# francescofugazzi/3dgsconverter

Hardware: NVIDIA H100
Metric: Msplats/s SOR k=16 (higher is better)
Workload: dtype f32

## Files before the change

### 3dgsconverter_b200/csrc/gsx_sor.cu

```cuda
#include "gsx_common.cuh"
#include "gsx_sor.cuh"

#include "gsx_radix.cuh"
#include <math.h>

namespace gsx {

#define GSX_D2LIM_BITS 0x60ad78ebu
#define GSX_FULL 0xffffffffu

constexpr int kMortonBits = 15;
constexpr float kMortonScale = (float)(1 << (kMortonBits / 3));
constexpr float kMortonMax = kMortonScale - 1.f;
constexpr int kSmallBucket = 64;
constexpr int kQueryBatch = 16;
constexpr int kMergeThreshold = 9;
constexpr int kKnnMinBlocks = 8;
constexpr int kFlatSupers = 8;
const char* sor_build_info() {
    return "knn=r02c;epi_smem=1;first_sort=1;query_batch=16;minblocks=8;merge_threshold=9;small_bucket=64;"
           "flat_supers=8;knn16=0;tma=0;i32=1";
}


SorWs sor_carve(void* ws, int64_t ws_bytes, int64_t n, size_t sort_ws_bytes) {
    SorWs w;
    Carver c(ws, (size_t)ws_bytes);
    int64_t nchunk = (n + 31) / 32, nsuper = (nchunk + 31) / 32;
    w.n = n;
    w.spos = c.take<float4>(n);
    w.tab_se = c.take<int2>(n);
    w.tab_box = c.take<float4>(2 * n);
    w.startbits = c.take<uint32_t>(nchunk);
    w.cellbits = c.take<uint32_t>(nchunk);
    w.bigbits = c.take<uint32_t>(nchunk);
    w.startlist = c.take<uint32_t>(n / 8 + 1024);
    w.caabb = c.take<float4>(2 * nchunk);
    w.saabb = c.take<float4>(2 * nsuper);
    w.partial = c.take<float>(6 * 1024);
    w.minmax = c.take<float>(8);
    w.counters = c.take<unsigned int>(64);
    w.stats = c.take<unsigned long long>(8);
    w.meanstd = c.take<float>(8);
    w.ms_bytes = mean_std_ws_bytes(n);
    w.ms_ws = c.take<char>(w.ms_bytes);
    w.grid_total = align_up(c.off, 256);
    w.keys0 = c.take<uint64_t>(n);
    w.keys1 = c.take<uint64_t>(n);
    w.sort_ws_bytes = sort_ws_bytes;
    w.sort_ws = c.take<char>(sort_ws_bytes);
    w.total = align_up(c.off, 256);
    w.ok = c.ok();
    w.grid_ok = w.grid_total <= (size_t)(ws_bytes > 0 ? ws_bytes : 0);
    return w;
}

size_t sor_sort_ws_bytes(int64_t n) { return radix_ws_bytes(n) + 256; }

int64_t sor_workspace_bytes(int64_t n) {
    if (n < 1) n = 1;
    SorWs w = sor_carve(nullptr, 0, n, sor_sort_ws_bytes(n));
    return (int64_t)w.total + 1024;
}

int64_t sor_grid_workspace_bytes(int64_t n) {
    if (n < 1) n = 1;
    SorWs w = sor_carve(nullptr, 0, n, sor_sort_ws_bytes(n));
    return (int64_t)w.grid_total;
}


__global__ void __launch_bounds__(256) k_minmax_partial(const float* __restrict__ xyz, int64_t n,
                                                        float* __restrict__ partial) {
    float lo[3] = {INFINITY, INFINITY, INFINITY}, hi[3] = {-INFINITY, -INFINITY, -INFINITY};
    int64_t stride = (int64_t)gridDim.x * blockDim.x;
    for (int64_t i = (int64_t)blockIdx.x * blockDim.x + threadIdx.x; i < n; i += stride) {
#pragma unroll
        for (int a = 0; a < 3; ++a) {
            float v = xyz[3 * i + a];
            lo[a] = fminf(lo[a], v);
            hi[a] = fmaxf(hi[a], v);
        }
    }
    __shared__ float sm[6][8];
#pragma unroll
    for (int a = 0; a < 3; ++a) {
#pragma unroll
        for (int o = 16; o > 0; o >>= 1) {
            lo[a] = fminf(lo[a], __shfl_xor_sync(GSX_FULL, lo[a], o));
            hi[a] = fmaxf(hi[a], __shfl_xor_sync(GSX_FULL, hi[a], o));
        }
        if (lane_id() == 0) {
            sm[a][threadIdx.x >> 5] = lo[a];
            sm[3 + a][threadIdx.x >> 5] = hi[a];
        }
    }
    __syncthreads();
    if (threadIdx.x < 6) {
        float r = sm[threadIdx.x][0];
        for (int w = 1; w < 8; ++w) r = threadIdx.x < 3 ? fminf(r, sm[threadIdx.x][w]) : fmaxf(r, sm[threadIdx.x][w]);
        partial[blockIdx.x * 6 + threadIdx.x] = r;
    }
}

__global__ void k_minmax_final(const float* __restrict__ partial, int nblocks, float* __restrict__ out) {
    const int a = threadIdx.x >> 5, lane = threadIdx.x & 31;
    if (a >= 6) return;
    float r = a < 3 ? INFINITY : -INFINITY;
    for (int b = lane; b < nblocks; b += 32) r = a < 3 ? fminf(r, partial[b * 6 + a]) : fmaxf(r, partial[b * 6 + a]);
#pragma unroll
    for (int o = 16; o > 0; o >>= 1) {
        float t = __shfl_xor_sync(GSX_FULL, r, o);
        r = a < 3 ? fminf(r, t) : fmaxf(r, t);
    }
    if (lane == 0) out[a] = r;
}

int sor_minmax(const float* xyz, int64_t n, float* minmax_dev, float* partial, cudaStream_t st) {
    int blocks = (int)((n + 255) / 256);
    int cap = sm_count() * 4;
    if (blocks > cap) blocks = cap;
    if (blocks > 1024) blocks = 1024;
    if (blocks < 1) blocks = 1;
    k_minmax_partial<<<blocks, 256, 0, st>>>(xyz, n, partial);
    GSX_KERNEL_CHECK();
    k_minmax_final<<<1, 192, 0, st>>>(partial, blocks, minmax_dev);
    GSX_KERNEL_CHECK();
    return GSX_OK;
}


__device__ __forceinline__ uint32_t spread6(uint32_t v) {
    v &= 63u;
    v = (v | (v << 8)) & 0x0000300Fu;
    v = (v | (v << 4)) & 0x000030C3u;
    v = (v | (v << 2)) & 0x00009249u;
    return v;
}

__device__ __forceinline__ uint32_t bucket_hash(float x, float y, float z, float bx, float by, float bz, float cell,
                                                int64_t n, uint64_t M64, float& fx, float& fy, float& fz, float& flx,
                                                float& fly, float& flz) {
    fx = __fdiv_rn(__fsub_rn(x, bx), cell);
    fy = __fdiv_rn(__fsub_rn(y, by), cell);
    fz = __fdiv_rn(__fsub_rn(z, bz), cell);
    flx = floorf(fx), fly = floorf(fy), flz = floorf(fz);
    int64_t gx = (int64_t)(int32_t)flx, gy = (int64_t)(int32_t)fly, gz = (int64_t)(int32_t)flz;
    int64_t hx = (gx * 73856093LL) ^ (gy * 19349663LL) ^ (gz * 83492791LL);
    int64_t h;
    if (hx >= 0) {
        uint64_t q = __umul64hi((uint64_t)hx, M64);
        uint64_t r = (uint64_t)hx - q * (uint64_t)n;
        while (r >= (uint64_t)n) r -= (uint64_t)n;
        h = (int64_t)r;
    } else {
        h = hx % n;
        if (h < 0) h += n;
    }
    return (uint32_t)h;
}

__device__ __forceinline__ uint32_t bucket_of(float x, float y, float z, float bx, float by, float bz, float cell,
                                              int64_t n, uint64_t M64) {
    float a, b, c, d, e, f;
    return bucket_hash(x, y, z, bx, by, bz, cell, n, M64, a, b, c, d, e, f);
}

__device__ __forceinline__ uint64_t bucket_key(float x, float y, float z, float bx, float by, float bz, float cell,
                                               int64_t n, uint64_t M64) {
    float fx, fy, fz, flx, fly, flz;
    const uint32_t h = bucket_hash(x, y, z, bx, by, bz, cell, n, M64, fx, fy, fz, flx, fly, flz);
    uint32_t sx = (uint32_t)fminf(kMortonMax, fmaxf(0.f, (fx - flx) * kMortonScale));
    uint32_t sy = (uint32_t)fminf(kMortonMax, fmaxf(0.f, (fy - fly) * kMortonScale));
    uint32_t sz = (uint32_t)fminf(kMortonMax, fmaxf(0.f, (fz - flz) * kMortonScale));
    uint32_t mort = (spread6(sx) << 2) | (spread6(sy) << 1) | spread6(sz);
    return ((uint64_t)h << kMortonBits) | (uint64_t)mort;
}

struct PackFmt {
    int idx_bits, mort_bits, bucket_bits;
    __host__ __device__ int key_shift() const { return idx_bits + mort_bits; }
    __host__ __device__ uint64_t idx_mask() const { return (1ull << idx_bits) - 1ull; }
    __host__ __device__ int sort_begin() const { return idx_bits; }
    __host__ __device__ int sort_end() const { return idx_bits + mort_bits + bucket_bits; }
};

static int bits_for(int64_t n) {
    int b = 1;
    while (((int64_t)1 << b) < n) ++b;
    return b;
}

static PackFmt pack_fmt(int64_t n_items, int64_t n_buckets) {
    PackFmt f;
    f.idx_bits = bits_for(n_items);
    f.bucket_bits = bits_for(n_buckets);
    int avail = 64 - f.idx_bits - f.bucket_bits;
    if (avail > kMortonBits) avail = kMortonBits;
    f.mort_bits = avail < 0 ? 0 : avail - avail % 3;
    return f;
}

__device__ __forceinline__ uint64_t pack_word(uint64_t key , uint64_t bucket_sub,
                                              int64_t idx, PackFmt f) {
    const uint64_t bucket = (key >> kMortonBits) - bucket_sub;
    const uint64_t mort = (key & ((1ull << kMortonBits) - 1ull)) >> (kMortonBits - f.mort_bits);
    return (((bucket << f.mort_bits) | mort) << f.idx_bits) | (uint64_t)idx;
}

__global__ void __launch_bounds__(256) k_sor_keys(const float* __restrict__ xyz, int64_t n, float bx, float by,
                                                  float bz, float cell, uint64_t M64, PackFmt f,
                                                  uint64_t* __restrict__ keys) {
    int64_t i = (int64_t)blockIdx.x * blockDim.x + threadIdx.x;
    if (i >= n) return;
    keys[i] = pack_word(bucket_key(xyz[3 * i], xyz[3 * i + 1], xyz[3 * i + 2], bx, by, bz, cell, n, M64), 0, i, f);
}

__device__ __forceinline__ uint32_t float_to_ord(float f) {
    const uint32_t u = __float_as_uint(f);
    return (u & 0x80000000u) ? ~u : (u | 0x80000000u);
}
__device__ __forceinline__ float ord_to_float(uint32_t o) {
    return __uint_as_float((o & 0x80000000u) ? (o & 0x7fffffffu) : ~o);
}

template <bool GATHER>
__device__ __forceinline__ void
    sor_finish_tile(const int64_t tile, const float* __restrict__ xyz, const uint64_t* __restrict__ keys, PackFmt fmt,
                    float4* __restrict__ spos, int64_t n, float bx, float by, float bz, float cell, uint64_t M64,
                    int2* __restrict__ tab_se, uint32_t* __restrict__ startbits, uint32_t* __restrict__ cellbits,
                    float4* __restrict__ caabb, float4* __restrict__ saabb) {
    const int64_t j = tile * 1024 + threadIdx.x;
    const int lane = lane_id();
    float lo[3] = {INFINITY, INFINITY, INFINITY}, hi[3] = {-INFINITY, -INFINITY, -INFINITY};
    uint32_t h = 0xffffffffu;
    auto hash_at = [&](int64_t t) -> uint32_t {
        if (GATHER) return (uint32_t)(keys[t] >> fmt.key_shift());
        const float4 q = spos[t];
        return bucket_of(q.x, q.y, q.z, bx, by, bz, cell, n, M64);
    };
    int gcx = 0x7fffffff, gcy = 0, gcz = 0;
    if (j < n) {
        float x, y, z;
        if (GATHER) {
            const uint64_t word = keys[j];
            const int32_t idx = (int32_t)(word & fmt.idx_mask());
            x = xyz[3 * (int64_t)idx], y = xyz[3 * (int64_t)idx + 1], z = xyz[3 * (int64_t)idx + 2];
            spos[j] = make_float4(x, y, z, __int_as_float(idx));
            h = (uint32_t)(word >> fmt.key_shift());
        } else {
            const float4 p = spos[j];
            x = p.x, y = p.y, z = p.z;
            h = bucket_of(x, y, z, bx, by, bz, cell, n, M64);
        }
        gcx = (int)floorf(__fdiv_rn(__fsub_rn(x, bx), cell));
        gcy = (int)floorf(__fdiv_rn(__fsub_rn(y, by), cell));
        gcz = (int)floorf(__fdiv_rn(__fsub_rn(z, bz), cell));
        lo[0] = hi[0] = x;
        lo[1] = hi[1] = y;
        lo[2] = hi[2] = z;
    }
    __shared__ uint32_t sh_h[1024];
    sh_h[threadIdx.x] = h;
    __syncthreads();
    uint32_t hprev = threadIdx.x > 0 ? sh_h[threadIdx.x - 1] : 0xffffffffu;
    uint32_t hnext = threadIdx.x < 1023 ? sh_h[threadIdx.x + 1] : 0xffffffffu;
    if (j < n) {
        if (threadIdx.x == 0 && j > 0) hprev = hash_at(j - 1);
        if (threadIdx.x == 1023 && j + 1 < n) hnext = hash_at(j + 1);
    }
    __shared__ int sh_c[3][1024];
    sh_c[0][threadIdx.x] = gcx, sh_c[1][threadIdx.x] = gcy, sh_c[2][threadIdx.x] = gcz;
    __syncthreads();
    const bool newcell = j < n && (threadIdx.x == 0 || sh_c[0][threadIdx.x - 1] != gcx ||
                                   sh_c[1][threadIdx.x - 1] != gcy || sh_c[2][threadIdx.x - 1] != gcz);
    const unsigned cb = __ballot_sync(GSX_FULL, newcell);
    const bool start = j < n && (j == 0 || h != hprev);
    const bool end = j < n && (j == n - 1 || h != hnext);
    if (start) tab_se[h].x = (int)j;
    if (end) tab_se[h].y = (int)(j + 1);
    const unsigned sb = __ballot_sync(GSX_FULL, start);
#pragma unroll
    for (int a = 0; a < 3; ++a) {
        lo[a] = ord_to_float(__reduce_min_sync(GSX_FULL, float_to_ord(lo[a])));
        hi[a] = ord_to_float(__reduce_max_sync(GSX_FULL, float_to_ord(hi[a])));
    }
    __shared__ float sm[6][32];
    const int w = threadIdx.x >> 5;
    const int64_t chunk = tile * 32 + w;
    if (lane == 0) {
        if (chunk * 32 < n) {
            startbits[chunk] = sb;
            cellbits[chunk] = cb;
            caabb[2 * chunk] = make_float4(lo[0], lo[1], lo[2], hi[0]);
            caabb[2 * chunk + 1] = make_float4(hi[1], hi[2], 0.f, 0.f);
        }
        for (int a = 0; a < 3; ++a) {
            sm[a][w] = lo[a];
            sm[3 + a][w] = hi[a];
        }
    }
    __syncthreads();
    if (w == 0) {
        float v[6];
#pragma unroll
        for (int a = 0; a < 6; ++a) {
            v[a] = sm[a][lane];
#pragma unroll
            for (int o = 16; o > 0; o >>= 1) {
                float t = __shfl_xor_sync(GSX_FULL, v[a], o);
                v[a] = a < 3 ? fminf(v[a], t) : fmaxf(v[a], t);
            }
        }
        if (lane == 0) {
            saabb[2 * tile] = make_float4(v[0], v[1], v[2], v[3]);
            saabb[2 * tile + 1] = make_float4(v[4], v[5], 0.f, 0.f);
        }
    }
}

template <bool GATHER>
__global__ void __launch_bounds__(1024)
    k_sor_finish(const float* __restrict__ xyz, const uint64_t* __restrict__ keys, PackFmt fmt,
                 float4* __restrict__ spos, int64_t n, float bx, float by, float bz, float cell, uint64_t M64,
                 int2* __restrict__ tab_se, uint32_t* __restrict__ startbits, uint32_t* __restrict__ cellbits,
                 float4* __restrict__ caabb, float4* __restrict__ saabb) {
    sor_finish_tile<GATHER>(blockIdx.x, xyz, keys, fmt, spos, n, bx, by, bz, cell, M64, tab_se, startbits, cellbits, caabb,
                            saabb);
}

__global__ void __launch_bounds__(1024)
    k_sor_finish_gated(float4* __restrict__ spos, int64_t n, float bx, float by, float bz, float cell, uint64_t M64,
                       int2* __restrict__ tab_se, uint32_t* __restrict__ startbits, uint32_t* __restrict__ cellbits,
                       float4* __restrict__ caabb, float4* __restrict__ saabb, const unsigned int* __restrict__ gate) {
    if (!*gate) return;
    const int64_t tiles = (n + 1023) / 1024;
    for (int64_t t = blockIdx.x; t < tiles; t += gridDim.x) {
        sor_finish_tile<false>(t, nullptr, nullptr, PackFmt{}, spos, n, bx, by, bz, cell, M64, tab_se, startbits, cellbits,
                               caabb, saabb);
        __syncthreads();
    }
}

__device__ __forceinline__ void bucket_box_partial(const float4* __restrict__ spos, const float4* __restrict__ caabb,
                                                   int64_t s, int64_t end, int lane, float (&lo)[3], float (&hi)[3]) {
    lo[0] = lo[1] = lo[2] = INFINITY;
    hi[0] = hi[1] = hi[2] = -INFINITY;
    int64_t cf = (s + 31) >> 5, cl = end >> 5;
    int64_t head_end = cf * 32, tail_begin = cl * 32;
    if (cf > cl) {
        head_end = end;
        tail_begin = end;
        cf = cl = 0;
    }
    for (int64_t t = s + lane; t < head_end; t += 32) {
        float4 p = spos[t];
        lo[0] = fminf(lo[0], p.x), lo[1] = fminf(lo[1], p.y), lo[2] = fminf(lo[2], p.z);
        hi[0] = fmaxf(hi[0], p.x), hi[1] = fmaxf(hi[1], p.y), hi[2] = fmaxf(hi[2], p.z);
    }
    for (int64_t c = cf + lane; c < cl; c += 32) {
        float4 a = caabb[2 * c], b = caabb[2 * c + 1];
        lo[0] = fminf(lo[0], a.x), lo[1] = fminf(lo[1], a.y), lo[2] = fminf(lo[2], a.z);
        hi[0] = fmaxf(hi[0], a.w), hi[1] = fmaxf(hi[1], b.x), hi[2] = fmaxf(hi[2], b.y);
    }
    for (int64_t t = tail_begin + lane; t < end; t += 32) {
        float4 p = spos[t];
        lo[0] = fminf(lo[0], p.x), lo[1] = fminf(lo[1], p.y), lo[2] = fminf(lo[2], p.z);
        hi[0] = fmaxf(hi[0], p.x), hi[1] = fmaxf(hi[1], p.y), hi[2] = fmaxf(hi[2], p.z);
    }
}

__device__ __forceinline__ void
    bucket_boxes_chunk(const int64_t chunk, const uint32_t* __restrict__ startbits, const float4* __restrict__ spos,
                       const float4* __restrict__ caabb, const int2* __restrict__ tab_se, int64_t n, float bx,
                       float by, float bz, float cell, uint64_t M64, float4* __restrict__ tab_box) {
    const int lane = lane_id();
    if (chunk * 32 >= n) return;
    unsigned m = startbits[chunk];
    uint32_t my_h = 0;
    int my_end = 0;
    if ((m >> lane) & 1u) {
        const float4 p0 = spos[chunk * 32 + lane];
        my_h = bucket_of(p0.x, p0.y, p0.z, bx, by, bz, cell, n, M64);
        my_end = tab_se[my_h].y;
    }
    while (m) {
        const int src = __ffs(m) - 1;
        m &= m - 1;
        const int64_t s = chunk * 32 + src;
        const uint32_t hb = __shfl_sync(GSX_FULL, my_h, src);
        const int64_t end = __shfl_sync(GSX_FULL, my_end, src);
        float lo[3], hi[3];
        bucket_box_partial(spos, caabb, s, end, lane, lo, hi);
#pragma unroll
        for (int a = 0; a < 3; ++a)
#pragma unroll
            for (int o = 16; o > 0; o >>= 1) {
                lo[a] = fminf(lo[a], __shfl_xor_sync(GSX_FULL, lo[a], o));
                hi[a] = fmaxf(hi[a], __shfl_xor_sync(GSX_FULL, hi[a], o));
            }
        if (lane == 0) {
            tab_box[2 * (size_t)hb] = make_float4(lo[0], lo[1], lo[2], 0.f);
            tab_box[2 * (size_t)hb + 1] = make_float4(hi[0], hi[1], hi[2], 0.f);
        }
    }
}

__global__ void __launch_bounds__(256)
    k_sor_bucket_boxes(const uint32_t* __restrict__ startbits, const float4* __restrict__ spos,
                       const float4* __restrict__ caabb, const int2* __restrict__ tab_se, int64_t n, float bx,
                       float by, float bz, float cell, uint64_t M64, float4* __restrict__ tab_box) {
    bucket_boxes_chunk(((int64_t)blockIdx.x * blockDim.x + threadIdx.x) >> 5, startbits, spos, caabb, tab_se, n, bx, by, bz,
                       cell, M64, tab_box);
}

__global__ void __launch_bounds__(256)
    k_sor_bucket_boxes_gated(const uint32_t* __restrict__ startbits, const float4* __restrict__ spos,
                             const float4* __restrict__ caabb, const int2* __restrict__ tab_se, int64_t n, float bx,
                             float by, float bz, float cell, uint64_t M64, float4* __restrict__ tab_box,
                             const unsigned int* __restrict__ gate) {
    if (!*gate) return;
    const int64_t nchunk = (n + 31) >> 5, step = ((int64_t)gridDim.x * blockDim.x) >> 5;
    for (int64_t c = ((int64_t)blockIdx.x * blockDim.x + threadIdx.x) >> 5; c < nchunk; c += step)
        bucket_boxes_chunk(c, startbits, spos, caabb, tab_se, n, bx, by, bz, cell, M64, tab_box);
}

struct StartList {
    unsigned int* count;
    unsigned int* pos;
    unsigned int capacity;
};

__global__ void __launch_bounds__(1024)
    k_sor_finish_flags(const float4* __restrict__ spos, const uint8_t* __restrict__ flags, int64_t n,
                       uint32_t* __restrict__ startbits, uint32_t* __restrict__ cellbits, float4* __restrict__ caabb,
                       float4* __restrict__ saabb, StartList sl) {
    const int64_t j = (int64_t)blockIdx.x * 1024 + threadIdx.x;
    const int lane = lane_id();
    float lo[3] = {INFINITY, INFINITY, INFINITY}, hi[3] = {-INFINITY, -INFINITY, -INFINITY};
    bool start = false, newcell = false;
    if (j < n) {
        const float4 p = spos[j];
        lo[0] = hi[0] = p.x;
        lo[1] = hi[1] = p.y;
        lo[2] = hi[2] = p.z;
        const uint8_t f = flags[j];
        start = (f & 1) != 0;
        newcell = (f & 2) != 0;
    }
    const unsigned sb = __ballot_sync(GSX_FULL, start), cb = __ballot_sync(GSX_FULL, newcell);
    __shared__ unsigned s_wcnt[32], s_base;
    const int w = threadIdx.x >> 5;
    if (lane == 0) s_wcnt[w] = __popc(sb);
#pragma unroll
    for (int a = 0; a < 3; ++a) {
        lo[a] = ord_to_float(__reduce_min_sync(GSX_FULL, float_to_ord(lo[a])));
        hi[a] = ord_to_float(__reduce_max_sync(GSX_FULL, float_to_ord(hi[a])));
    }
    __shared__ float sm[6][32];
    const int64_t chunk = (int64_t)blockIdx.x * 32 + w;
    if (lane == 0) {
        if (chunk * 32 < n) {
            startbits[chunk] = sb;
            cellbits[chunk] = cb;
            caabb[2 * chunk] = make_float4(lo[0], lo[1], lo[2], hi[0]);
            caabb[2 * chunk + 1] = make_float4(hi[1], hi[2], 0.f, 0.f);
        }
        for (int a = 0; a < 3; ++a) {
            sm[a][w] = lo[a];
            sm[3 + a][w] = hi[a];
        }
    }
    __syncthreads();
    if (w == 0) {
        unsigned v = s_wcnt[lane], x = v;
#pragma unroll
        for (int o = 1; o < 32; o <<= 1) {
            unsigned y = __shfl_up_sync(GSX_FULL, x, o);
            if (lane >= o) x += y;
        }
        s_wcnt[lane] = x - v;
        if (lane == 31) {
            unsigned base = 0;
            if (x) {
                base = atomicAdd(sl.count, x);
                if (base + x > sl.capacity) {
                    atomicExch(sl.count + 1, 1u);
                    base = 0xffffffffu;
                }
            }
            s_base = base;
        }
        float vb[6];
#pragma unroll
        for (int a = 0; a < 6; ++a) {
            vb[a] = sm[a][lane];
#pragma unroll
            for (int o = 16; o > 0; o >>= 1) {
                float t = __shfl_xor_sync(GSX_FULL, vb[a], o);
                vb[a] = a < 3 ? fminf(vb[a], t) : fmaxf(vb[a], t);
            }
        }
        if (lane == 0) {
            saabb[2 * (int64_t)blockIdx.x] = make_float4(vb[0], vb[1], vb[2], vb[3]);
            saabb[2 * (int64_t)blockIdx.x + 1] = make_float4(vb[4], vb[5], 0.f, 0.f);
        }
    }
    __syncthreads();
    if (start && s_base != 0xffffffffu)
        sl.pos[s_base + s_wcnt[w] + __popc(sb & ((1u << lane) - 1u))] = (unsigned)j;
}

__global__ void __launch_bounds__(256)
    k_sor_bucket_tail(const float4* __restrict__ spos, const uint8_t* __restrict__ flags, int64_t n, float bx, float by,
                      float bz, float cell, uint64_t M64, int2* __restrict__ tab_se, float4* __restrict__ tab_box,
                      uint32_t* __restrict__ bigbits, StartList sl) {
    if (sl.count[1]) return;
    const unsigned t = blockIdx.x * blockDim.x + threadIdx.x;
    if (t >= sl.count[0]) return;
    const int64_t pj = sl.pos[t];
    const float4 p = spos[pj];
    const uint32_t h = bucket_of(p.x, p.y, p.z, bx, by, bz, cell, n, M64);
    float blo[3] = {p.x, p.y, p.z}, bhi[3] = {p.x, p.y, p.z};
    int64_t u = pj + 1;
    const int64_t lim = pj + kSmallBucket < n ? pj + kSmallBucket : n;
    for (; u < lim; ++u) {
        if (flags[u] & 1) break;
        const float4 c = spos[u];
        blo[0] = fminf(blo[0], c.x), blo[1] = fminf(blo[1], c.y), blo[2] = fminf(blo[2], c.z);
        bhi[0] = fmaxf(bhi[0], c.x), bhi[1] = fmaxf(bhi[1], c.y), bhi[2] = fmaxf(bhi[2], c.z);
    }
    const bool closed = u == n || (flags[u] & 1);
    if (closed) {
        tab_se[h] = make_int2((int)pj, (int)u);
        tab_box[2 * (size_t)h] = make_float4(blo[0], blo[1], blo[2], 0.f);
        tab_box[2 * (size_t)h + 1] = make_float4(bhi[0], bhi[1], bhi[2], 0.f);
    } else {
        tab_se[h].x = (int)pj;
        atomicOr(bigbits + (pj >> 5), 1u << (pj & 31));
    }
}

__global__ void __launch_bounds__(256)
    k_sor_big_buckets(const uint32_t* __restrict__ bigbits, const uint32_t* __restrict__ startbits,
                      const float4* __restrict__ spos, const float4* __restrict__ caabb, int64_t n, float bx, float by,
                      float bz, float cell, uint64_t M64, int2* __restrict__ tab_se, float4* __restrict__ tab_box,
                      StartList sl) {
    if (sl.count[1]) return;
    const int lane = lane_id();
    const int64_t nchunk = (n + 31) >> 5;
    const int64_t wstep = (((int64_t)gridDim.x * blockDim.x) >> 5) * 32;
    for (int64_t c0 = (((int64_t)blockIdx.x * blockDim.x + threadIdx.x) >> 5) * 32; c0 < nchunk; c0 += wstep) {
    const uint32_t myword = c0 + lane < nchunk ? bigbits[c0 + lane] : 0u;
    unsigned wordmask = __ballot_sync(GSX_FULL, myword != 0u);
    while (wordmask) {
    const int wl = __ffs(wordmask) - 1;
    wordmask &= wordmask - 1;
    const int64_t chunk = c0 + wl;
    unsigned m = __shfl_sync(GSX_FULL, myword, wl);
    while (m) {
        const int src = __ffs(m) - 1;
        m &= m - 1;
        const int64_t s = chunk * 32 + src;
        int64_t end = n;
        {
            const unsigned rest = src == 31 ? 0u : (startbits[chunk] & (0xffffffffu << (src + 1)));
            if (rest) {
                end = chunk * 32 + __ffs(rest) - 1;
            } else {
                for (int64_t d0 = chunk + 1; d0 < nchunk; d0 += 32) {
                    const int64_t c = d0 + lane;
                    const unsigned wv = c < nchunk ? startbits[c] : 0u;
                    const unsigned any = __ballot_sync(GSX_FULL, wv != 0u);
                    if (any) {
                        const int l = __ffs(any) - 1;
                        const unsigned word = __shfl_sync(GSX_FULL, wv, l);
                        end = (d0 + l) * 32 + __ffs(word) - 1;
                        break;
                    }
                }
            }
        }
        const float4 p0 = spos[s];
        const uint32_t hb = bucket_of(p0.x, p0.y, p0.z, bx, by, bz, cell, n, M64);
        float lo[3], hi[3];
        bucket_box_partial(spos, caabb, s, end, lane, lo, hi);
#pragma unroll
        for (int a = 0; a < 3; ++a) {
            lo[a] = ord_to_float(__reduce_min_sync(GSX_FULL, float_to_ord(lo[a])));
            hi[a] = ord_to_float(__reduce_max_sync(GSX_FULL, float_to_ord(hi[a])));
        }
        if (lane == 0) {
            tab_se[hb].y = (int)end;
            tab_box[2 * (size_t)hb] = make_float4(lo[0], lo[1], lo[2], 0.f);
            tab_box[2 * (size_t)hb + 1] = make_float4(hi[0], hi[1], hi[2], 0.f);
        }
    }
    }
    }
}

template <bool GATHER>
static int sor_finish(const float* xyz, int64_t n, const float* bmin, float cell, SorWs& w, PackFmt fmt, cudaStream_t st) {
    const uint64_t M64 = 0xFFFFFFFFFFFFFFFFull / (uint64_t)n;
    GSX_CUDA_CHECK(cudaMemsetAsync(w.tab_se, 0, (size_t)n * sizeof(int2), st));
    k_sor_finish<GATHER><<<(int)((n + 1023) / 1024), 1024, 0, st>>>(xyz, w.keys_sorted, fmt, w.spos, n, bmin[0],
                                                                    bmin[1], bmin[2], cell, M64, w.tab_se, w.startbits,
                                                                    w.cellbits, w.caabb, w.saabb);
    GSX_KERNEL_CHECK();
    k_sor_bucket_boxes<<<(int)((n + 255) / 256), 256, 0, st>>>(w.startbits, w.spos, w.caabb, w.tab_se, n, bmin[0],
                                                               bmin[1], bmin[2], cell, M64, w.tab_box);
    GSX_KERNEL_CHECK();
    return GSX_OK;
}

int sor_build(const float* xyz, int64_t n, const float* bmin, float cell, SorWs& w, cudaStream_t st) {
    GSX_NVTX("gsx::sor_build");
    int blocks = (int)((n + 255) / 256);
    const PackFmt fmt = pack_fmt(n, n);
    k_sor_keys<<<blocks, 256, 0, st>>>(xyz, n, bmin[0], bmin[1], bmin[2], cell, 0xFFFFFFFFFFFFFFFFull / (uint64_t)n,
                                       fmt, w.keys0);
    GSX_KERNEL_CHECK();
    {
        int rc = radix_sort_keys(w.keys0, w.keys1, n, fmt.sort_begin(), fmt.sort_end(), w.sort_ws, w.sort_ws_bytes,
                                 &w.keys_sorted, st);
        if (rc) return rc;
    }
    return sor_finish<true>(xyz, n, bmin, cell, w, fmt, st);
}


__global__ void __launch_bounds__(256) k_sor_owner_keys(const float* __restrict__ xyz, int64_t n, int64_t n_global,
                                                        int world, float bx, float by, float bz, float cell,
                                                        uint64_t M64, int idx_bits, uint64_t* __restrict__ keys) {
    int64_t i = (int64_t)blockIdx.x * blockDim.x + threadIdx.x;
    if (i >= n) return;
    uint64_t h = bucket_key(xyz[3 * i], xyz[3 * i + 1], xyz[3 * i + 2], bx, by, bz, cell, n_global, M64) >> kMortonBits;
    keys[i] = (((h * (uint64_t)world) / (uint64_t)n_global) << idx_bits) | (uint64_t)i;
}

__global__ void __launch_bounds__(256) k_sor_gather_slab(const float* __restrict__ xyz,
                                                         const uint64_t* __restrict__ words, uint64_t idx_mask, int64_t n,
                                                         int64_t idx_base, float4* __restrict__ pos4) {
    int64_t j = (int64_t)blockIdx.x * blockDim.x + threadIdx.x;
    if (j >= n) return;
    int32_t idx = (int32_t)(words[j] & idx_mask);
    pos4[j] = make_float4(xyz[3 * (int64_t)idx], xyz[3 * (int64_t)idx + 1], xyz[3 * (int64_t)idx + 2],
                          __int_as_float((int)(idx_base + idx)));
}

__global__ void k_sor_owner_counts(const uint64_t* __restrict__ owners_sorted, int idx_bits, int64_t n, int world,
                                   long long* __restrict__ cuts) {
    int o = threadIdx.x;
    if (o > world) return;
    int64_t lo = 0, hi = n;
    while (lo < hi) {
        int64_t mid = (lo + hi) >> 1;
        if ((owners_sorted[mid] >> idx_bits) < (uint64_t)o) lo = mid + 1; else hi = mid;
    }
    cuts[o] = lo;
}

int sor_dist_local_run(const float* xyz, int64_t n_local, int64_t idx_base, int64_t n_global, int world,
                       const float* bmin, float cell, float4* pos4_out, long long* cuts_dev, SorWs& w,
                       cudaStream_t st) {
    GSX_NVTX("gsx::sor_dist_local_run");
    GSX_REQUIRE(world >= 1 && world <= 255, GSX_ERR_ARG, "sor: world size must be in [1,255]");
    if (n_local == 0) {
        GSX_CUDA_CHECK(cudaMemsetAsync(cuts_dev, 0, (size_t)(world + 1) * sizeof(long long), st));
        return GSX_OK;
    }
    int blocks = (int)((n_local + 255) / 256);
    const int idx_bits = bits_for(n_local);
    k_sor_owner_keys<<<blocks, 256, 0, st>>>(xyz, n_local, n_global, world, bmin[0], bmin[1], bmin[2], cell,
                                             0xFFFFFFFFFFFFFFFFull / (uint64_t)n_global, idx_bits, w.keys0);
    GSX_KERNEL_CHECK();
    uint64_t* ks = nullptr;
    int rc = radix_sort_keys(w.keys0, w.keys1, n_local, idx_bits, idx_bits + 8, w.sort_ws, w.sort_ws_bytes, &ks,
                             st);
    if (rc) return rc;
    k_sor_gather_slab<<<blocks, 256, 0, st>>>(xyz, ks, (1ull << idx_bits) - 1ull, n_local, idx_base, pos4_out);
    GSX_KERNEL_CHECK();
    k_sor_owner_counts<<<1, 256, 0, st>>>(ks, idx_bits, n_local, world, cuts_dev);
    GSX_KERNEL_CHECK();
    return GSX_OK;
}

__global__ void __launch_bounds__(256) k_gather4(const float4* __restrict__ in, const uint64_t* __restrict__ words,
                                                 uint64_t idx_mask, int64_t n, float4* __restrict__ out) {
    int64_t j = (int64_t)blockIdx.x * blockDim.x + threadIdx.x;
    if (j < n) out[j] = in[words[j] & idx_mask];
}

__global__ void __launch_bounds__(256) k_sor_keys_pos4(const float4* __restrict__ pos4, int64_t n, int64_t n_global,
                                                       float bx, float by, float bz, float cell, uint64_t M64,
                                                       uint64_t bucket_lo, PackFmt f, uint64_t* __restrict__ keys) {
    int64_t i = (int64_t)blockIdx.x * blockDim.x + threadIdx.x;
    if (i >= n) return;
    float4 p = pos4[i];
    keys[i] = pack_word(bucket_key(p.x, p.y, p.z, bx, by, bz, cell, n_global, M64), bucket_lo, i, f);
}

__global__ void __launch_bounds__(256)
    k_owner_gather_flags(const float4* __restrict__ in, const uint64_t* __restrict__ keys_sorted, PackFmt fmt, int64_t m, float bx, float by, float bz, float cell,
                         float4* __restrict__ out, uint8_t* __restrict__ flags) {
    const int64_t j = (int64_t)blockIdx.x * blockDim.x + threadIdx.x;
    __shared__ int sh_c[3][256];
    int gx = 0x7fffffff, gy = 0, gz = 0;
    float4 p = make_float4(0.f, 0.f, 0.f, 0.f);
    if (j < m) {
        p = in[keys_sorted[j] & fmt.idx_mask()];
        out[j] = p;
        gx = (int)floorf(__fdiv_rn(__fsub_rn(p.x, bx), cell));
        gy = (int)floorf(__fdiv_rn(__fsub_rn(p.y, by), cell));
        gz = (int)floorf(__fdiv_rn(__fsub_rn(p.z, bz), cell));
    }
    sh_c[0][threadIdx.x] = gx, sh_c[1][threadIdx.x] = gy, sh_c[2][threadIdx.x] = gz;
    __syncthreads();
    if (j >= m) return;
    const bool start = j == 0 || (keys_sorted[j] >> fmt.key_shift()) != (keys_sorted[j - 1] >> fmt.key_shift());
    bool newcell = threadIdx.x == 0 || sh_c[0][threadIdx.x - 1] != gx || sh_c[1][threadIdx.x - 1] != gy ||
                   sh_c[2][threadIdx.x - 1] != gz;
    flags[j] = (uint8_t)((start ? 1 : 0) | ((newcell || start) ? 2 : 0));
}

int sor_dist_merge(const float4* pos4_in, int64_t m, int64_t n_global, int64_t bucket_lo, int64_t bucket_hi,
                   const float* bmin, float cell, float4* pos4_out, uint8_t* flags_out, SorWs& w, cudaStream_t st) {
    GSX_NVTX("gsx::sor_dist_merge");
    if (m == 0) return GSX_OK;
    GSX_REQUIRE(bucket_lo >= 0 && bucket_lo < bucket_hi && bucket_hi <= n_global, GSX_ERR_ARG, "sor: bad bucket range");
    int blocks = (int)((m + 255) / 256);
    const PackFmt fmt = pack_fmt(m, bucket_hi - bucket_lo);
    k_sor_keys_pos4<<<blocks, 256, 0, st>>>(pos4_in, m, n_global, bmin[0], bmin[1], bmin[2], cell,
                                            0xFFFFFFFFFFFFFFFFull / (uint64_t)n_global, (uint64_t)bucket_lo, fmt, w.keys0);
    GSX_KERNEL_CHECK();
    uint64_t* ks = nullptr;
    int rc = radix_sort_keys(w.keys0, w.keys1, m, fmt.sort_begin(), fmt.sort_end(), w.sort_ws, w.sort_ws_bytes, &ks, st);
    if (rc) return rc;
    if (flags_out)
        k_owner_gather_flags<<<blocks, 256, 0, st>>>(pos4_in, ks, fmt, m, bmin[0], bmin[1], bmin[2], cell, pos4_out,
                                                     flags_out);
    else
        k_gather4<<<blocks, 256, 0, st>>>(pos4_in, ks, fmt.idx_mask(), m, pos4_out);
    GSX_KERNEL_CHECK();
    return GSX_OK;
}

int sor_build_from_sorted(const float4* spos_in, const uint8_t* flags, int64_t n, const float* bmin, float cell, SorWs& w,
                          cudaStream_t st) {
    GSX_NVTX("gsx::sor_build_from_sorted");
    if (spos_in != w.spos)
        GSX_CUDA_CHECK(cudaMemcpyAsync(w.spos, spos_in, (size_t)n * sizeof(float4), cudaMemcpyDeviceToDevice, st));
    w.keys_sorted = nullptr;
    if (!flags) return sor_finish<false>(nullptr, n, bmin, cell, w, PackFmt{}, st);
    const uint64_t M64 = 0xFFFFFFFFFFFFFFFFull / (uint64_t)n;
    const int64_t nchunk = (n + 31) / 32;
    StartList sl;
    sl.count = w.counters + 8;
    sl.pos = reinterpret_cast<unsigned int*>(w.startlist);
    sl.capacity = (unsigned)(n / 8 + 1024);
    GSX_CUDA_CHECK(cudaMemsetAsync(w.tab_se, 0, (size_t)n * sizeof(int2), st));
    GSX_CUDA_CHECK(cudaMemsetAsync(w.bigbits, 0, (size_t)nchunk * sizeof(uint32_t), st));
    GSX_CUDA_CHECK(cudaMemsetAsync(sl.count, 0, 2 * sizeof(unsigned int), st));
    k_sor_finish_flags<<<(int)((n + 1023) / 1024), 1024, 0, st>>>(w.spos, flags, n, w.startbits, w.cellbits, w.caabb,
                                                                  w.saabb, sl);
    GSX_KERNEL_CHECK();
    const unsigned tail_blocks = (sl.capacity + 255) / 256;
    k_sor_bucket_tail<<<tail_blocks, 256, 0, st>>>(w.spos, flags, n, bmin[0], bmin[1], bmin[2], cell, M64, w.tab_se,
                                                   w.tab_box, w.bigbits, sl);
    GSX_KERNEL_CHECK();
    k_sor_big_buckets<<<sm_count() * 8, 256, 0, st>>>(w.bigbits, w.startbits, w.spos, w.caabb, n, bmin[0], bmin[1], bmin[2],
                                                      cell, M64, w.tab_se, w.tab_box, sl);
    GSX_KERNEL_CHECK();
    const int resident = sm_count() * 2;
    k_sor_finish_gated<<<resident, 1024, 0, st>>>(w.spos, n, bmin[0], bmin[1], bmin[2], cell, M64, w.tab_se, w.startbits,
                                                  w.cellbits, w.caabb, w.saabb, sl.count + 1);
    GSX_KERNEL_CHECK();
    k_sor_bucket_boxes_gated<<<resident * 4, 256, 0, st>>>(w.startbits, w.spos, w.caabb, w.tab_se, n, bmin[0], bmin[1],
                                                           bmin[2], cell, M64, w.tab_box, sl.count + 1);
    GSX_KERNEL_CHECK();
    return GSX_OK;
}


__device__ __forceinline__ uint32_t probe_hash(int nx, int ny, int nz, uint32_t n, uint64_t M, int mode) {
    if (mode == GSX_HASH_MODE_I32WRAP) {
        int32_t h = (int32_t)((uint32_t)nx * 73856093u) ^ (int32_t)((uint32_t)ny * 19349663u) ^
                    (int32_t)((uint32_t)nz * 83492791u);
        uint32_t a = h < 0 ? (uint32_t)(-(int64_t)h) : (uint32_t)h;
        uint32_t r = fastmod_u32(a, M, n);
        return h < 0 ? (r ? n - r : 0u) : r;
    } else {
        int64_t h = ((int64_t)nx * 73856093LL) ^ ((int64_t)ny * 19349663LL) ^ ((int64_t)nz * 83492791LL);
        int64_t r = h % (int64_t)n;
        if (r < 0) r += n;
        return (uint32_t)r;
    }
}

__device__ __forceinline__ float box_lb(const float4* __restrict__ aabb, int64_t id, float qx, float qy, float qz) {
    float4 a = __ldg(aabb + 2 * id), b = __ldg(aabb + 2 * id + 1);
    float dx = fmaxf(fmaxf(__fsub_rn(a.x, qx), __fsub_rn(qx, a.w)), 0.f);
    float dy = fmaxf(fmaxf(__fsub_rn(a.y, qy), __fsub_rn(qy, b.x)), 0.f);
    float dz = fmaxf(fmaxf(__fsub_rn(a.z, qz), __fsub_rn(qz, b.y)), 0.f);
    return __fadd_rn(__fadd_rn(__fmul_rn(dx, dx), __fmul_rn(dy, dy)), __fmul_rn(dz, dz));
}

__device__ __forceinline__ float cmpx(float v, int j, bool take_min) {
    float o = __shfl_xor_sync(GSX_FULL, v, j);
    return take_min ? fminf(v, o) : fmaxf(v, o);
}

__device__ __forceinline__ float warp_sort32(float v, int lane) {
#pragma unroll
    for (int k = 2; k <= 32; k <<= 1) {
#pragma unroll
        for (int j = k >> 1; j > 0; j >>= 1) v = cmpx(v, j, ((lane & k) == 0) == ((lane & j) == 0));
    }
    return v;
}

template <int NREG>
struct TopK {
    float v0, v1;
    float tau;
    int K;
    __device__ __forceinline__ void init(int k) {
        K = k;
        v0 = v1 = tau = __uint_as_float(GSX_D2LIM_BITS);
    }
    __device__ __forceinline__ void refresh_tau() {
        tau = (NREG == 2 && K > 32) ? __shfl_sync(GSX_FULL, v1, K - 33) : __shfl_sync(GSX_FULL, v0, K - 1);
    }
    __device__ __forceinline__ void insert(float x, int lane) {
        float up0 = __shfl_up_sync(GSX_FULL, v0, 1);
        if (NREG == 2) {
            float top0 = __shfl_sync(GSX_FULL, v0, 31);
            float up1 = __shfl_up_sync(GSX_FULL, v1, 1);
            if (lane == 0) up1 = top0;
            if (v1 > x) v1 = fmaxf(up1, x);
        }
        if (lane == 0) up0 = 0.f;
        if (v0 > x) v0 = fmaxf(up0, x);
        refresh_tau();
    }
    __device__ __forceinline__ void merge32(float nv, int lane) {
        nv = warp_sort32(nv, lane);
        if (__all_sync(GSX_FULL, v0 == __uint_as_float(GSX_D2LIM_BITS))) {
            v0 = nv;
            refresh_tau();
            return;
        }
        float r = __shfl_sync(GSX_FULL, nv, 31 - lane);
        float m = fminf(v0, r);
#pragma unroll
        for (int j = 16; j > 0; j >>= 1) m = cmpx(m, j, (lane & j) == 0);
        v0 = m;
        refresh_tau();
    }
};

typedef int pos_t;

template <int NREG, bool STATS>
__device__ __forceinline__ void scan32(const float4* __restrict__ spos, pos_t j, bool valid, float qx, float qy,
                                       float qz, TopK<NREG>& tk, int lane, unsigned long long& n_scanned) {
    float d2 = INFINITY;
    if (valid) {
        float4 c = __ldg(spos + j);
        float ax = __fsub_rn(qx, c.x), ay = __fsub_rn(qy, c.y), az = __fsub_rn(qz, c.z);
        d2 = __fadd_rn(__fadd_rn(__fmul_rn(ax, ax), __fmul_rn(ay, ay)), __fmul_rn(az, az));
    }
    if (STATS) n_scanned += __popc(__ballot_sync(GSX_FULL, valid));
    bool pass = valid && d2 > 1.0e-12f && d2 < tk.tau;
    unsigned m = __ballot_sync(GSX_FULL, pass);
    if (NREG == 1 && __popc(m) >= kMergeThreshold) {
        tk.merge32(pass ? d2 : __uint_as_float(GSX_D2LIM_BITS), lane);
        return;
    }
    while (m) {
        int src = __ffs(m) - 1;
        m &= m - 1;
        float x = __shfl_sync(GSX_FULL, d2, src);
        if (x < tk.tau) tk.insert(x, lane);
    }
}

template <int NREG, bool STATS, int ES>
__global__ void __launch_bounds__(256, kKnnMinBlocks)
    k_sor_knn(const float4* __restrict__ spos, const int2* __restrict__ tab_se, const float4* __restrict__ tab_box,
              const uint32_t* __restrict__ cellbits, const float4* __restrict__ caabb,
              const float4* __restrict__ saabb, float* __restrict__ final_means, unsigned int* __restrict__ work,
              int64_t q_begin, int64_t q_end, int q_stride, int q_phase, int K, int hash_mode, float bx, float by,
              float bz, float cell,
              uint32_t n, uint64_t M, unsigned long long* __restrict__ stats) {
    const int lane = lane_id();
    unsigned long long st_visits = 0, st_scanned = 0, st_boxes = 0, st_queries = 0;
    static_assert(ES >= 0 && ES <= 33, "a row holds at most the 32 ranks of one register + the row number");
    extern __shared__ float s_epi[];
    float* const epi = s_epi + (threadIdx.x >> 5) * (kQueryBatch * (ES > 0 ? ES : 1));
    const int pdx = lane / 9 - 1, pdy = (lane / 3) % 3 - 1, pdz = lane % 3 - 1;

    for (;;) {
        unsigned int b0 = 0;
        if (lane == 0) b0 = atomicAdd(work, (unsigned)kQueryBatch);
        b0 = __shfl_sync(GSX_FULL, b0, 0);
        int64_t qb = q_begin + ((int64_t)(b0 / kQueryBatch) * q_stride + q_phase) * kQueryBatch;
        if (qb >= q_end) break;
        int64_t qe = qb + kQueryBatch < q_end ? qb + kQueryBatch : q_end;
        const uint32_t cellword = __ldg(cellbits + (qb >> 5));
        int ps = 0, pc = 0;
        float blx = 0.f, bly = 0.f, blz = 0.f, bhx = 0.f, bhy = 0.f, bhz = 0.f;
        const pos_t qb_p = (pos_t)qb, qe_p = (pos_t)qe;
#pragma unroll 1
        for (pos_t i = qb_p; i < qe_p; ++i) {
            const float4 q = __ldg(spos + i);
            const uint32_t w_i = (i >> 5) == (qb_p >> 5) ? cellword : __ldg(cellbits + (i >> 5));
            if (i == qb_p || ((w_i >> (i & 31)) & 1u)) {
                const int gx = (int)floorf(__fdiv_rn(__fsub_rn(q.x, bx), cell));
                const int gy = (int)floorf(__fdiv_rn(__fsub_rn(q.y, by), cell));
                const int gz = (int)floorf(__fdiv_rn(__fsub_rn(q.z, bz), cell));
                ps = 0, pc = 0;
                if (lane < 27) {
                    uint32_t h = probe_hash(gx + pdx, gy + pdy, gz + pdz, n, M, hash_mode);
                    const int2 se = __ldg(tab_se + h);
                    ps = se.x;
                    pc = se.y - se.x;
                    if (pc > 0) {
                        const float4 b0 = __ldg(tab_box + 2 * (size_t)h), b1 = __ldg(tab_box + 2 * (size_t)h + 1);
                        blx = b0.x, bly = b0.y, blz = b0.z, bhx = b1.x, bhy = b1.y, bhz = b1.z;
                    }
                }
            }
            if (STATS) {
// ... 188 lines not shown
```

Before: 1083.

## Reorder large-bucket points within each 1024 tile by kd-split for tighter chunk boxes

Adds a kernel that, for each 1024-point tile, finds buckets larger than the small-bucket threshold and recursively splits them along the widest axis into 32-aligned halves. It uses per-axis bitonic sorts and stable partitions in shared memory, then rewrites spos and recomputes cell bits and chunk/super AABBs. Tighter chunk boxes should let the kNN query for SOR prune more candidate chunks. The cost is an extra kernel pass with about 60KB of dynamic shared memory, which tiles without large buckets exit early. The cell-change and box computation is moved into a shared helper that uses warp shuffles instead of a 1024-entry shared array.

```diff
diff --git a/3dgsconverter_b200/csrc/gsx_sor.cu b/3dgsconverter_b200/csrc/gsx_sor.cu
--- a/3dgsconverter_b200/csrc/gsx_sor.cu
+++ b/3dgsconverter_b200/csrc/gsx_sor.cu
@@ -19,7 +19,7 @@
 constexpr int kFlatSupers = 8;
 const char* sor_build_info() {
     return "knn=r02c;epi_smem=1;first_sort=1;query_batch=16;minblocks=8;merge_threshold=9;small_bucket=64;"
-           "flat_supers=8;knn16=0;tma=0;i32=1";
+           "flat_supers=8;knn16=0;tma=0;i32=1;order=kd_super";
 }
 
 
@@ -224,6 +224,65 @@
     return __uint_as_float((o & 0x80000000u) ? (o & 0x7fffffffu) : ~o);
 }
 
+__device__ __forceinline__ void tile_cells_boxes(const int64_t tile, const bool valid, const float x, const float y,
+                                                 const float z, int64_t n, float bx, float by, float bz, float cell,
+                                                 uint32_t* __restrict__ cellbits, float4* __restrict__ caabb,
+                                                 float4* __restrict__ saabb) {
+    const int lane = lane_id(), w = threadIdx.x >> 5;
+    float lo[3] = {INFINITY, INFINITY, INFINITY}, hi[3] = {-INFINITY, -INFINITY, -INFINITY};
+    int gcx = 0x7fffffff, gcy = 0, gcz = 0;
+    if (valid) {
+        gcx = (int)floorf(__fdiv_rn(__fsub_rn(x, bx), cell));
+        gcy = (int)floorf(__fdiv_rn(__fsub_rn(y, by), cell));
+        gcz = (int)floorf(__fdiv_rn(__fsub_rn(z, bz), cell));
+        lo[0] = hi[0] = x;
+        lo[1] = hi[1] = y;
+        lo[2] = hi[2] = z;
+    }
+    int px = __shfl_up_sync(GSX_FULL, gcx, 1), py = __shfl_up_sync(GSX_FULL, gcy, 1), pz = __shfl_up_sync(GSX_FULL, gcz, 1);
+    __shared__ int sh_c[3][32];
+    if (lane == 31) sh_c[0][w] = gcx, sh_c[1][w] = gcy, sh_c[2][w] = gcz;
+    __syncthreads();
+    if (lane == 0 && w > 0) px = sh_c[0][w - 1], py = sh_c[1][w - 1], pz = sh_c[2][w - 1];
+    const bool newcell = valid && (threadIdx.x == 0 || px != gcx || py != gcy || pz != gcz);
+    const unsigned cb = __ballot_sync(GSX_FULL, newcell);
+#pragma unroll
+    for (int a = 0; a < 3; ++a) {
+        lo[a] = ord_to_float(__reduce_min_sync(GSX_FULL, float_to_ord(lo[a])));
+        hi[a] = ord_to_float(__reduce_max_sync(GSX_FULL, float_to_ord(hi[a])));
+    }
+    __shared__ float sm[6][32];
+    const int64_t chunk = tile * 32 + w;
+    if (lane == 0) {
+        if (chunk * 32 < n) {
+            cellbits[chunk] = cb;
+            caabb[2 * chunk] = make_float4(lo[0], lo[1], lo[2], hi[0]);
+            caabb[2 * chunk + 1] = make_float4(hi[1], hi[2], 0.f, 0.f);
+        }
+        for (int a = 0; a < 3; ++a) {
+            sm[a][w] = lo[a];
+            sm[3 + a][w] = hi[a];
+        }
+    }
+    __syncthreads();
+    if (w == 0) {
+        float v[6];
+#pragma unroll
+        for (int a = 0; a < 6; ++a) {
+            v[a] = sm[a][lane];
+#pragma unroll
+            for (int o = 16; o > 0; o >>= 1) {
+                float t = __shfl_xor_sync(GSX_FULL, v[a], o);
+                v[a] = a < 3 ? fminf(v[a], t) : fmaxf(v[a], t);
+            }
+        }
+        if (lane == 0) {
+            saabb[2 * tile] = make_float4(v[0], v[1], v[2], v[3]);
+            saabb[2 * tile + 1] = make_float4(v[4], v[5], 0.f, 0.f);
+        }
+    }
+}
+
 template <bool GATHER>
 __device__ __forceinline__ void
     sor_finish_tile(const int64_t tile, const float* __restrict__ xyz, const uint64_t* __restrict__ keys, PackFmt fmt,
@@ -232,16 +291,14 @@
                     float4* __restrict__ caabb, float4* __restrict__ saabb) {
     const int64_t j = tile * 1024 + threadIdx.x;
     const int lane = lane_id();
-    float lo[3] = {INFINITY, INFINITY, INFINITY}, hi[3] = {-INFINITY, -INFINITY, -INFINITY};
     uint32_t h = 0xffffffffu;
     auto hash_at = [&](int64_t t) -> uint32_t {
         if (GATHER) return (uint32_t)(keys[t] >> fmt.key_shift());
         const float4 q = spos[t];
         return bucket_of(q.x, q.y, q.z, bx, by, bz, cell, n, M64);
     };
-    int gcx = 0x7fffffff, gcy = 0, gcz = 0;
+    float x = 0.f, y = 0.f, z = 0.f;
     if (j < n) {
-        float x, y, z;
         if (GATHER) {
             const uint64_t word = keys[j];
             const int32_t idx = (int32_t)(word & fmt.idx_mask());
@@ -253,12 +310,6 @@
             x = p.x, y = p.y, z = p.z;
             h = bucket_of(x, y, z, bx, by, bz, cell, n, M64);
         }
-        gcx = (int)floorf(__fdiv_rn(__fsub_rn(x, bx), cell));
-        gcy = (int)floorf(__fdiv_rn(__fsub_rn(y, by), cell));
-        gcz = (int)floorf(__fdiv_rn(__fsub_rn(z, bz), cell));
-        lo[0] = hi[0] = x;
-        lo[1] = hi[1] = y;
-        lo[2] = hi[2] = z;
     }
     __shared__ uint32_t sh_h[1024];
     sh_h[threadIdx.x] = h;
@@ -269,54 +320,14 @@
         if (threadIdx.x == 0 && j > 0) hprev = hash_at(j - 1);
         if (threadIdx.x == 1023 && j + 1 < n) hnext = hash_at(j + 1);
     }
-    __shared__ int sh_c[3][1024];
-    sh_c[0][threadIdx.x] = gcx, sh_c[1][threadIdx.x] = gcy, sh_c[2][threadIdx.x] = gcz;
-    __syncthreads();
-    const bool newcell = j < n && (threadIdx.x == 0 || sh_c[0][threadIdx.x - 1] != gcx ||
-                                   sh_c[1][threadIdx.x - 1] != gcy || sh_c[2][threadIdx.x - 1] != gcz);
-    const unsigned cb = __ballot_sync(GSX_FULL, newcell);
     const bool start = j < n && (j == 0 || h != hprev);
     const bool end = j < n && (j == n - 1 || h != hnext);
     if (start) tab_se[h].x = (int)j;
     if (end) tab_se[h].y = (int)(j + 1);
     const unsigned sb = __ballot_sync(GSX_FULL, start);
-#pragma unroll
-    for (int a = 0; a < 3; ++a) {
-        lo[a] = ord_to_float(__reduce_min_sync(GSX_FULL, float_to_ord(lo[a])));
-        hi[a] = ord_to_float(__reduce_max_sync(GSX_FULL, float_to_ord(hi[a])));
-    }
-    __shared__ float sm[6][32];
-    const int w = threadIdx.x >> 5;
-    const int64_t chunk = tile * 32 + w;
-    if (lane == 0) {
-        if (chunk * 32 < n) {
-            startbits[chunk] = sb;
-            cellbits[chunk] = cb;
-            caabb[2 * chunk] = make_float4(lo[0], lo[1], lo[2], hi[0]);
-            caabb[2 * chunk + 1] = make_float4(hi[1], hi[2], 0.f, 0.f);
-        }
-        for (int a = 0; a < 3; ++a) {
-            sm[a][w] = lo[a];
-            sm[3 + a][w] = hi[a];
-        }
-    }
-    __syncthreads();
-    if (w == 0) {
-        float v[6];
-#pragma unroll
-        for (int a = 0; a < 6; ++a) {
-            v[a] = sm[a][lane];
-#pragma unroll
-            for (int o = 16; o > 0; o >>= 1) {
-                float t = __shfl_xor_sync(GSX_FULL, v[a], o);
-                v[a] = a < 3 ? fminf(v[a], t) : fmaxf(v[a], t);
-            }
-        }
-        if (lane == 0) {
-            saabb[2 * tile] = make_float4(v[0], v[1], v[2], v[3]);
-            saabb[2 * tile + 1] = make_float4(v[4], v[5], 0.f, 0.f);
-        }
-    }
+    const int64_t chunk = tile * 32 + (threadIdx.x >> 5);
+    if (lane == 0 && chunk * 32 < n) startbits[chunk] = sb;
+    tile_cells_boxes(tile, j < n, x, y, z, n, bx, by, bz, cell, cellbits, caabb, saabb);
 }
 
 template <bool GATHER>
@@ -600,6 +611,175 @@
     }
 }
 
+
+template <int NF>
+__device__ __forceinline__ void block_excl_count(const bool (&f)[NF], int (&r)[NF], int* s_w) {
+    const int lane = lane_id(), w = threadIdx.x >> 5;
+    unsigned b[NF];
+#pragma unroll
+    for (int i = 0; i < NF; ++i) {
+        b[i] = __ballot_sync(GSX_FULL, f[i]);
+        if (lane == 0) s_w[i * 32 + w] = __popc(b[i]);
+    }
+    __syncthreads();
+    if (w < NF) {
+        const int v = s_w[w * 32 + lane];
+        int x = v;
+#pragma unroll
+        for (int o = 1; o < 32; o <<= 1) {
+            const int y = __shfl_up_sync(GSX_FULL, x, o);
+            if (lane >= o) x += y;
+        }
+        s_w[w * 32 + lane] = x - v;
+    }
+    __syncthreads();
+#pragma unroll
+    for (int i = 0; i < NF; ++i) r[i] = s_w[i * 32 + w] + __popc(b[i] & ((1u << lane) - 1u));
+    __syncthreads();
+}
+
+__device__ __forceinline__ void block_sort1024x3(uint64_t (&v)[3], uint64_t* s_key) {
+    const int t = threadIdx.x;
+#pragma unroll
+    for (int k = 2; k <= 1024; k <<= 1) {
+#pragma unroll
+        for (int d = k >> 1; d > 0; d >>= 1) {
+            uint64_t o[3];
+            if (d >= 32) {
+#pragma unroll
+                for (int a = 0; a < 3; ++a) s_key[a * 1024 + t] = v[a];
+                __syncthreads();
+#pragma unroll
+                for (int a = 0; a < 3; ++a) o[a] = s_key[a * 1024 + (t ^ d)];
+                __syncthreads();
+            } else {
+#pragma unroll
+                for (int a = 0; a < 3; ++a) o[a] = __shfl_xor_sync(GSX_FULL, v[a], d);
+            }
+            const bool lo = ((t & k) == 0) == ((t & d) == 0);
+#pragma unroll
+            for (int a = 0; a < 3; ++a) v[a] = lo ? (v[a] < o[a] ? v[a] : o[a]) : (v[a] > o[a] ? v[a] : o[a]);
+        }
+    }
+}
+
+__device__ __forceinline__ float axis_of(const float4& p, int a) { return a == 0 ? p.x : (a == 1 ? p.y : p.z); }
+
+struct KdSmem {
+    float4 pt[1024];
+    uint64_t key[3][1024];
+    uint16_t list[2][3][1024];
+    uint8_t flag[1024];
+    int w[3 * 32];
+};
+
+__global__ void __launch_bounds__(1024)
+    k_sor_kd_supers(float4* __restrict__ spos, int64_t n, float bx, float by, float bz, float cell, uint64_t M64,
+                    const int2* __restrict__ tab_se, const uint32_t* __restrict__ startbits,
+                    uint32_t* __restrict__ cellbits, float4* __restrict__ caabb, float4* __restrict__ saabb) {
+    extern __shared__ __align__(16) unsigned char kd_smem_raw[];
+    KdSmem& S = *reinterpret_cast<KdSmem*>(kd_smem_raw);
+    const int t = threadIdx.x, lane = lane_id();
+    const int64_t tile = blockIdx.x, j = tile * 1024 + t;
+    const bool valid = j < n;
+    const float4 p = valid ? spos[j] : make_float4(0.f, 0.f, 0.f, 0.f);
+    S.pt[t] = p;
+    const bool pstart = valid && (t == 0 || ((startbits[j >> 5] >> lane) & 1u));
+    int piece;
+    {
+        const bool f[1] = {pstart};
+        int r[1];
+        block_excl_count<1>(f, r, S.w);
+        piece = r[0] + (pstart ? 0 : -1);
+    }
+    int2* const s_piece = reinterpret_cast<int2*>(&S.key[0][0]);
+    if (pstart) {
+        const int2 se = tab_se[bucket_of(p.x, p.y, p.z, bx, by, bz, cell, n, M64)];
+        const int64_t end = (int64_t)se.y - tile * 1024;
+        s_piece[piece] = make_int2(t, (int)(end < 1024 ? end : 1024) | (se.y - se.x > kSmallBucket ? (int)0x80000000 : 0));
+    }
+    __syncthreads();
+    int na = 0, nb = 0;
+    bool active = false;
+    if (valid) {
+        const int2 pc = s_piece[piece];
+        active = pc.y < 0;
+        na = pc.x, nb = pc.y & 0x7fffffff;
+    }
+    if (!__syncthreads_or(active)) return;
+    {
+        uint64_t key[3];
+#pragma unroll
+        for (int a = 0; a < 3; ++a)
+            key[a] = !valid ? ((1ull << 63) | (uint64_t)t)
+                            : ((uint64_t)piece << 42) | ((active ? (uint64_t)float_to_ord(axis_of(p, a)) : 0ull) << 10) |
+                                  (uint64_t)t;
+        block_sort1024x3(key, &S.key[0][0]);
+#pragma unroll
+        for (int a = 0; a < 3; ++a) S.list[0][a][t] = (uint16_t)(key[a] & 1023u);
+    }
+    int cur = 0;
+#pragma unroll 1
+    for (;;) {
+        const bool split = active && (((na >> 5) + 1) << 5) < nb;
+        if (!__syncthreads_or(split)) break;
+        int m = 0;
+        if (split) {
+            int ax = 0;
+            float best = -1.f;
+#pragma unroll
+            for (int a = 0; a < 3; ++a) {
+                const float e = __fsub_rn(axis_of(S.pt[S.list[cur][a][nb - 1]], a), axis_of(S.pt[S.list[cur][a][na]], a));
+                if (e > best) best = e, ax = a;
+            }
+            const int first = ((na >> 5) + 1) << 5, last = ((nb - 1) >> 5) << 5;
+            m = ((((na + nb) >> 1) + 16) >> 5) << 5;
+            m = m < first ? first : (m > last ? last : m);
+            S.flag[S.list[cur][ax][t]] = t < m;
+        }
+        __syncthreads();
+        int id[3], c[3];
+        bool f[3];
+#pragma unroll
+        for (int a = 0; a < 3; ++a) {
+            id[a] = S.list[cur][a][t];
+            f[a] = split && S.flag[id[a]];
+        }
+        block_excl_count<3>(f, c, S.w);
+        int* const s_cnt = reinterpret_cast<int*>(&S.key[0][0]);
+#pragma unroll
+        for (int a = 0; a < 3; ++a) s_cnt[a * 1024 + t] = c[a];
+        __syncthreads();
+#pragma unroll
+        for (int a = 0; a < 3; ++a) {
+            int dst = t;
+            if (split) {
+                const int left_before = c[a] - s_cnt[a * 1024 + na];
+                dst = f[a] ? na + left_before : m + (t - na) - left_before;
+            }
+            S.list[cur ^ 1][a][dst] = (uint16_t)id[a];
+        }
+        cur ^= 1;
+        if (split) {
+            if (t < m) nb = m;
+            else na = m;
+        }
+    }
+    __syncthreads();
+    const float4 q = S.pt[S.list[cur][0][t]];
+    if (active) spos[j] = q;
+    tile_cells_boxes(tile, valid, q.x, q.y, q.z, n, bx, by, bz, cell, cellbits, caabb, saabb);
+}
+
+static int sor_kd_order(int64_t n, const float* bmin, float cell, SorWs& w, cudaStream_t st) {
+    GSX_CUDA_CHECK(cudaFuncSetAttribute(k_sor_kd_supers, cudaFuncAttributeMaxDynamicSharedMemorySize, (int)sizeof(KdSmem)));
+    k_sor_kd_supers<<<(int)((n + 1023) / 1024), 1024, sizeof(KdSmem), st>>>(w.spos, n, bmin[0], bmin[1], bmin[2], cell,
+                                                               0xFFFFFFFFFFFFFFFFull / (uint64_t)n, w.tab_se, w.startbits,
+                                                               w.cellbits, w.caabb, w.saabb);
+    GSX_KERNEL_CHECK();
+    return GSX_OK;
+}
+
 template <bool GATHER>
 static int sor_finish(const float* xyz, int64_t n, const float* bmin, float cell, SorWs& w, PackFmt fmt, cudaStream_t st) {
     const uint64_t M64 = 0xFFFFFFFFFFFFFFFFull / (uint64_t)n;
@@ -611,7 +791,7 @@
     k_sor_bucket_boxes<<<(int)((n + 255) / 256), 256, 0, st>>>(w.startbits, w.spos, w.caabb, w.tab_se, n, bmin[0],
                                                                bmin[1], bmin[2], cell, M64, w.tab_box);
     GSX_KERNEL_CHECK();
-    return GSX_OK;
+    return sor_kd_order(n, bmin, cell, w, st);
 }
 
 int sor_build(const float* xyz, int64_t n, const float* bmin, float cell, SorWs& w, cudaStream_t st) {
@@ -779,7 +959,7 @@
     k_sor_bucket_boxes_gated<<<resident * 4, 256, 0, st>>>(w.startbits, w.spos, w.caabb, w.tab_se, n, bmin[0], bmin[1],
                                                            bmin[2], cell, M64, w.tab_box, sl.count + 1);
     GSX_KERNEL_CHECK();
-    return GSX_OK;
+    return sor_kd_order(n, bmin, cell, w, st);
 }
 
 
```

Result: faster. 1108, median of 6 (+2.3%).
